# SaeedRahmani/MPC-RL_for_AVs

Hardware: AMD Instinct MI355X
Metric: MPC solves/sec (horizon=20, batch=4096) (higher is better)
Workload: dtype f64

## Files before the change

### mpc-rl_for_avs_amd/csrc/mpc_engine.hip

```cpp
#include <hip/hip_runtime.h>

#include <atomic>
#include <chrono>
#include <cmath>
#include <cstdio>
#include <cstring>
#include <new>
#include <string>
#include <vector>

#include "../../include/mpc_mi355x.h"
#include "mpc_core.hpp"
#include "mpc_ltv.hpp"
#include "mpc_wave.hpp"
#include "mpc_wave_dev.hpp"
#include "mpc_preamble.hpp"
#include "mpc_preamble_wave.hpp"
#include "mpc_synth_env.hpp"
#include "mpc_rollout_glue.hpp"

namespace {

thread_local std::string g_last_error;

int fail(int code, const std::string &msg) {
    g_last_error = msg;
    return code;
}

#define HIP_TRY(expr)                                                                              \
    do {                                                                                           \
        hipError_t e_ = (expr);                                                                    \
        if (e_ != hipSuccess)                                                                      \
            return fail(MPC_ERR_HIP, std::string(#expr) + ": " + hipGetErrorString(e_));          \
    } while (0)

constexpr int kBlock = 64;
constexpr int kMaxDevices = 64;
constexpr int kWaveOcc = 3, kWaveOccGeneric = 3;
constexpr int kWaveOccGenericCC = 2;
constexpr int kWaveOccLat = 2, kLatDepth = 4;
constexpr int kRelaxLat = 7;

template <int NC, int RELAX = 0>
struct WaveCtx : mpc::wave::WaveOpsT<RELAX> {
    static constexpr int kN = NC;
    const double *table;
    int e0, M;
    __device__ __forceinline__ WaveCtx(mpc::wave::lds_double_t *l, const double *t, int e, int m)
        : mpc::wave::WaveOpsT<RELAX>{l}, table(t), e0(e), M(m) {}
    __device__ __forceinline__ void tick(int) const {}
    __device__ __forceinline__ double ref(int k, int c) const {
        int idx = e0 + k;
        idx = idx > M - 1 ? M - 1 : idx;
        idx = idx < 0 ? 0 : idx;
        return table[idx * mpc::REF_COLS + c];
    }
    __device__ __forceinline__ double refv(int k) const {
        int idx = e0 + k;
        idx = idx > M - 1 ? M - 1 : idx;
        idx = idx < 0 ? 0 : idx;
        return table[M * mpc::REF_COLS + idx];
    }
};

template <bool CC, class CTX>
__device__ __forceinline__ void stage_problem(CTX &ctx, const mpc::SolveParams &P, int b, int lane, int N, int SL,
                                              const double *__restrict__ ref5, int M, const double *__restrict__ vref,
                                              const double *__restrict__ others, int Vin) {
    const int OTH = SL * (N + 1) + mpc::wave::SC_SIZE;
    for (int node = lane; node <= N; node += kBlock) {
        double rv;
        if (vref) {
            rv = vref[(size_t)b * (N + 1) + node];
        } else {
            int idx = ctx.e0 + node;
            idx = idx > M - 1 ? M - 1 : idx;
            idx = idx < 0 ? 0 : idx;
            rv = ref5[M * mpc::REF_COLS + idx];
        }
        ctx.st(node * SL + mpc::wave::W_RV, rv);
    }
    if (CC && lane < P.V) {
        const double *ov = others + ((size_t)b * Vin + lane) * 4;
        const double sp = ov[2] * P.dt, hh = ov[3];
        ctx.st(OTH + lane * 4 + 0, ov[0]);
        ctx.st(OTH + lane * 4 + 1, ov[1]);
        ctx.st(OTH + lane * 4 + 2, sp * cos(hh));
        ctx.st(OTH + lane * 4 + 3, sp * sin(hh));
    }
}

template <bool CC, int NC, int OCC, int RELAX>
__global__ __launch_bounds__(kBlock, OCC) void mpc_solve_wave_kernel(
    mpc::SolveParams P, int B, const double *__restrict__ ref5, int M, const double *__restrict__ state,
    const int32_t *__restrict__ ego_index, const double *__restrict__ vref, const double *__restrict__ weights,
    const uint8_t *__restrict__ is_collide, const double *__restrict__ others, int Vin,
    const int32_t *__restrict__ nveh, double w_collision, const double *u_init, int u_shift, uint8_t *u_valid,
    double *__restrict__ u0_out, double *U_out, double *__restrict__ X_out, int32_t *__restrict__ status_out,
// ... 1486 lines not shown
```

### mpc-rl_for_avs_amd/csrc/mpc_wave.hpp

```cpp
#pragma once

#include "mpc_core.hpp"

namespace mpc {
namespace wave {

constexpr int kLanes = 64;
constexpr int kTrials = 4;
constexpr double kProjKeep = 0.1;
constexpr double kProjKeepEnd = 1e-3, kProjEndMu = 1e-6;
constexpr int kGnWatch = 4, kGnSkip = 4;
constexpr double kGnEndMu = 1e-2;
constexpr int kDwProbe = 4;
constexpr int kBoostIter = 28;
constexpr double kOpenLoopStep = 1e-9;
constexpr double kAcceptableTol = 1e-6;
constexpr int kAcceptableIter = 15;
constexpr double kRegMax = 1.0;
constexpr double kKappaEps = 30.0;
constexpr double kMinSlack = 1e-14;
constexpr double kInitPush = 1e-2;

enum : int {
    W_X = 0,
// ... 7 lines not shown
    W_KX = 36,
    W_KP = 44,
    W_KF = 48,
    W_RV = 50,
    W_ONE = 51,
    W_DTC = 52,
    W_SLOTS = 53,
    W_LX = 53,
    W_Q = 55,
    W_QG = 58,
    W_ZW = 61,
    W_WJ = 62,
    W_CROSS = 63,
    W_SLOTS_CC = 65
};
constexpr int kZeroWord = W_LIN + 2;
enum : int { LIN_A02 = 0, LIN_A12 = 1, LIN_A03 = 4, LIN_A13 = 5, LIN_A23 = 6, LIN_B01 = 8, LIN_B11 = 9, LIN_B21 = 10 };
enum : int { W_DXY = W_LX, W_GW = W_Q, W_DZW = W_Q + 1 };
static_assert(kTrials == 4, "the trial areas below are laid out for four trials");
MPC_HD constexpr int trial_x(bool, int t, int TB) { return t == 0 ? TB : (t == 1 ? W_LIN : (t == 2 ? W_LIN + 6 : W_KX)); }
MPC_HD constexpr int trial_u(bool cc, int t, int TB) { return trial_x(cc, t, TB); }
enum : int {
    SC_SPARE = 0,
    SC_TRIG = 4,
    SC_LOG = SC_TRIG + kTrigWords,
    SC_BND = SC_LOG + kLogWords,
    SC_K = SC_BND + 8,
    SC_NB = SC_K + 6,
    SC_SIZE = SC_NB + 3
};
enum : int { K_SF = 0, K_RD, K_RC, K_QTT, K_Q33, K_MUMIN };
constexpr int kMaxHorizon = kLanes;
enum : int {
    A_L00 = W_KX + 0, A_L01 = W_KX + 1, A_L11 = W_KX + 2, A_H22 = W_KX + 3, A_H23 = W_KX + 4, A_H33 = W_KX + 5,
    A_WTD = W_KX + 6, A_WVD = W_KX + 7, A_H66 = W_KP + 0, A_H77 = W_KP + 1, A_HV6 = W_KP + 2, A_HV7 = W_KF + 0,
    A_HV4 = W_KF + 1,
    A_HV0 = W_X,
    A_HV5 = W_U
};

constexpr int kPreSlots = 12;
enum : int { PQ = 0, PB = 8 };
constexpr double kNoBound = 1e300;

MPC_HD constexpr int stage_slots(bool cc) { return (cc ? W_SLOTS_CC : W_SLOTS) + kPreSlots; }
MPC_HD constexpr int lds_doubles(bool cc, int N, int V) { return stage_slots(cc) * (N + 1) + SC_SIZE + (cc ? 4 * V : 0); }

enum : int {
    T_PREP = 0, T_ADJOINT, T_DUALRES, T_RIC_INIT, T_RIC_SCALARS, T_RIC_L1, T_RIC_L2, T_RIC_2X2, T_RIC_L4, T_LINEAR,
    T_RATIOS, T_ROLL_DYN, T_ROLL_COST, T_DUALUPD,
    T_R_FEEDBACK, T_R_CLAMP, T_R_DYN, T_R_STORE, T_R_CHECK, T_R_PROJ, T_R_LDSW, T_COUNT
};
template <class CTX, class = void>
struct fine_ticks { static constexpr bool value = false; };
template <class CTX>
struct fine_ticks<CTX, decltype((void)CTX::kFine)> { static constexpr bool value = CTX::kFine; };

template <class T>
struct PerLane {
#if defined(__HIPCC__)
    T v;
    MPC_HD T &at(int) { return v; }
#else
    T v[kLanes];
    MPC_HD T &at(int lane) { return v[lane]; }
#endif
};

MPC_HD bool ratio_greater(double n2, double d2, double n1, double d1) {
    const double a = n2 * d1, b = n1 * d2;
    return a > b || (a == b && d2 > d1);
}

#if !defined(__HIPCC__)
inline int row_partner(int l, int step) {
    return step == 0 ? (l ^ 1) : (step == 1 ? (l ^ 2) : (step == 2 ? ((l & ~7) | (7 - (l & 7))) : ((l & ~15) | (15 - (l & 15)))));
}
template <class T, class OP>
inline void host_row_reduce(PerLane<T> &p, OP op) {
    for (int step = 0; step < 4; ++step) {
        T nv[kLanes];
        for (int l = 0; l < kLanes; ++l) nv[l] = op(p.v[l], p.v[row_partner(l, step)]);
        for (int l = 0; l < kLanes; ++l) p.v[l] = nv[l];
    }
}
template <class T, class OP>
inline T host_reduce(PerLane<T> &p, OP op) {
    host_row_reduce(p, op);
    return op(op(p.v[0], p.v[16]), op(p.v[32], p.v[48]));
}
#endif

MPC_HD constexpr int stage_transition_word(int r, int c, int lin, int zero, int one, int dtw) {
    const int key = 8 * r + c;
    int w = zero;
    w = (r < 4 && r == c) ? one : w;
    w = key == 8 * 4 + 6 ? one : w;
    w = key == 8 * 5 + 7 ? one : w;
    w = key == 8 * 0 + 2 ? lin + 0 : w;
    w = key == 8 * 0 + 3 ? lin + 1 : w;
    w = key == 8 * 1 + 2 ? lin + 2 : w;
    w = key == 8 * 1 + 3 ? lin + 3 : w;
    w = key == 8 * 2 + 3 ? lin + 4 : w;
    w = key == 8 * 3 + 6 ? dtw : w;
    w = key == 8 * 0 + 7 ? lin + 5 : w;
    w = key == 8 * 1 + 7 ? lin + 6 : w;
// ... 15 lines not shown
    MPC_HD double RC() const { return sc(SC_K + K_RC); }
    MPC_HD double WS() const { return c.fresh(ws_); }
    MPC_HD double WC() const { return c.fresh(wc_); }
    MPC_HD double WD() const { return c.fresh(wd_); }
    MPC_HD double WCOLL() const { return c.fresh(wcoll); }

    MPC_HD Solver(const SolveParams &P_, CTX &c_, const double *x0_, double ws, double wc, double wd, double wcl)
        : P(P_), c(c_), N(CTX::kN > 0 ? CTX::kN : P_.N), SL(stage_slots(CC)), SCR(SL * (N + 1)), OTH(SCR + SC_SIZE),
          dt(P_.dt), ws_(c_.uni(ws)), wc_(c_.uni(wc)), wd_(c_.uni(wd)), wcoll(c_.uni(wcl)) {
        x0[0] = x0_[0]; x0[1] = x0_[1]; x0[2] = x0_[2]; x0[3] = x0_[3];
    }
    MPC_HD double S(int k, int slot) const { return c.ld(k * SL + slot); }
    MPC_HD void S(int k, int slot, double v) { c.st(k * SL + slot, v); }
    MPC_HD double sc(int i) const { return c.ld(SCR + i); }
    MPC_HD void sc(int i, double v) { c.st(SCR + i, v); }
    MPC_HD double oth(int j, int q) const { return c.ld(OTH + j * 4 + q); }
    MPC_HD double xlo(int i) const { return sc(SC_BND + 0 + 2 * i); }
    MPC_HD double xhi(int i) const { return sc(SC_BND + 1 + 2 * i); }
    MPC_HD double ulo(int i) const { return sc(SC_BND + 4 + 2 * i); }
    MPC_HD double uhi(int i) const { return sc(SC_BND + 5 + 2 * i); }
    MPC_HD double flog(double x) const {
        double K[kLogWords];
        for (int i = 0; i < kLogWords; ++i) K[i] = sc(SC_LOG + i);
        return log_pos(K, x);
    }
    MPC_HD TrigCoef trig() const {
        TrigCoef K;
        for (int i = 0; i < 6; ++i) {
            K.s[i] = sc(SC_TRIG + i);
            K.c[i] = sc(SC_TRIG + 6 + i);
        }
        return K;
    }

    PerLane<double> red_a, red_b, red_c, red_w;
    PerLane<int> ls_feas;
    int any_wall = 0;
    MPC_HD int f_word(int r, int c) const {
        const int w = stage_transition_word(r, c, 0, 1000, 1001, 1002);
        int t = w;
        t = w == 1000 ? kZeroWord : t;
        t = w == 1001 ? W_ONE : t;
        t = w == 1002 ? W_DTC : t;
        t = w == 0 ? W_LIN + LIN_A02 : t;
        t = w == 1 ? W_LIN + LIN_A03 : t;
        t = w == 2 ? W_LIN + LIN_A12 : t;
        t = w == 3 ? W_LIN + LIN_A13 : t;
        t = w == 4 ? W_LIN + LIN_A23 : t;
        t = w == 5 ? W_LIN + LIN_B01 : t;
        t = w == 6 ? W_LIN + LIN_B11 : t;
        t = w == 7 ? W_LIN + LIN_B21 : t;
        return t;
    }
    PerLane<int> r_a, r_b, r_lxx, r_lux, r_m, r_lx, r_lu, r_kx;
    MPC_HD void set_roles4(int AB) {
        c.lanes([&](int lane_) {
            const int lane = c.opaque(lane_);
            const int hi = lane >> 4, blk = (lane >> 2) & 3, lo = lane & 3;
            const int zero = kZeroWord;
            r_a.at(lane_) = f_word(hi, lo);
            r_b.at(lane_) = f_word(hi, lo < 2 ? 6 + lo : 4);
            const int a = hi < lo ? hi : lo, b = hi < lo ? lo : hi;
            const int key = a * 4 + b;
            int slot = zero;
            slot = key == 0 * 4 + 0 ? A_L00 : slot;
            slot = key == 0 * 4 + 1 ? A_L01 : slot;
            slot = key == 1 * 4 + 1 ? A_L11 : slot;
            slot = key == 2 * 4 + 2 ? A_H22 : slot;
            slot = key == 2 * 4 + 3 ? A_H23 : slot;
            slot = key == 3 * 4 + 3 ? A_H33 : slot;
            r_lxx.at(lane_) = slot;
            r_lux.at(lane_) = hi == 1 ? (lo == 2 ? A_WTD : (lo == 3 ? A_WVD : zero)) : zero;
            r_m.at(lane_) = (hi == 0 && lo == 0) ? A_H66 : ((hi == 1 && lo == 1) ? A_H77 : zero);
            r_lx.at(lane_) = lo == 0 ? AB + A_HV0 + hi : zero;
            r_lu.at(lane_) = lo == 0 ? (hi == 0 ? A_HV6 : (hi == 1 ? A_HV7 : zero)) : zero;
            int out = -1;
            out = (blk == 0 && hi < 2) ? W_KX + 2 * lo + hi : out;
            out = (blk == 1 && hi < 2 && lo < 2) ? W_KP + 2 * lo + hi : out;
            out = (blk == 2 && hi < 2 && lo == 0) ? W_KF + hi : out;
            r_kx.at(lane_) = out;
        });
    }

    MPC_HD void load_stage4(int k, int AB, PerLane<double> &RA, PerLane<double> &RB, PerLane<double> &QXX, PerLane<double> &QUX,
                            PerLane<double> &M, PerLane<double> &QX, PerLane<double> &QU, double &lp0, double &lp1) {
        c.lanes([&](int lane) {
            const int base = k * SL;
            auto word = [&](int w) { return c.ld(base + w); };
            RA.at(lane) = word(r_a.at(lane));
            RB.at(lane) = word(r_b.at(lane));
            QXX.at(lane) = word(r_lxx.at(lane));
            QUX.at(lane) = word(r_lux.at(lane));
            M.at(lane) = word(r_m.at(lane));
            QX.at(lane) = word(r_lx.at(lane));
            QU.at(lane) = word(r_lu.at(lane));
        });
        lp0 = S(k, A_HV4);
        lp1 = S(k, AB + A_HV5);
    }
    MPC_HD bool sweep4(int CB, int AB, double mu, double delta_w, bool gn, double &dV1) {
        double tsig[2], tgr[2];
        for (int i = 0; i < 2; ++i) {
            const double xi = S(N, CB + W_X + 2 + i);
            const double rl = frcp(xi - xlo(i)), ru = frcp(xhi(i) - xi);
            tsig[i] = S(N, W_ZXL + i) * rl + S(N, W_ZXU + i) * ru + delta_w;
            tgr[i] = mu * (ru - rl);
        }
        PerLane<double> PXX, PXP, PX;
        c.lanes([&](int lane_) {
            const int lane = c.opaque_shared(lane_);
            const int hi = lane >> 4, lo = lane & 3;
            PXX.at(lane_) = hi == lo ? (hi == 2 ? tsig[0] : (hi == 3 ? tsig[1] : delta_w)) : 0.0;
            PXP.at(lane_) = 0.0;
            PX.at(lane_) = lo == 0 ? (hi == 2 ? tgr[0] : (hi == 3 ? tgr[1] : 0.0)) : 0.0;
        });
        double pp00 = 0.0, pp01 = 0.0, pp11 = 0.0, ppv0 = 0.0, ppv1 = 0.0;
        c.tick(T_RIC_INIT);
        const double rd_full = RD();
#pragma unroll 1
        for (int k = N - 1; k >= 0; --k) {
            const double rdk = (k >= 1) ? rd_full : 0.0;
            PerLane<double> RA, RB, QXX, QUX, M, QX, QU, T0, T1;
            double lp0, lp1;
            load_stage4(k, AB, RA, RB, QXX, QUX, M, QX, QU, lp0, lp1);
            c.lanes([&](int lane) {
                T0.at(lane) = 0.0;
// ... 67 lines not shown
                            q11 = S(k, W_QG + 2) - S(k, W_Q + 2);
                            if (any_wall && S(k, W_WJ) >= 0.0) {
                                q00 += 2.0 * S(k, W_ZW);
                                q11 += 2.0 * S(k, W_ZW);
                            }
                        }
                    }
                }
                c.lanes([&](int lane_) {
                    const int lane = c.opaque_shared(lane_);
                    const int hi = lane >> 4, lo = lane & 3;
                    const int a = hi < lo ? hi : lo, b = hi < lo ? lo : hi;
                    double cx = 0.0;
                    switch (a * 4 + b) {
                        case 0 * 4 + 0: cx = q00; break;
                        case 0 * 4 + 1: cx = q01; break;
                        case 1 * 4 + 1: cx = q11; break;
                        case 2 * 4 + 2: cx = -wtt; break;
                        case 2 * 4 + 3: cx = -wtv; break;
                        default: break;
                    }
                    QXX.at(lane_) += cx;
                    QUX.at(lane_) += hi == 1 ? (lo == 2 ? -wtd : (lo == 3 ? -wvd : 0.0)) : 0.0;
                });
                hc -= wdd;
                det = ha * hc - hb * hb;
                pd = (ha > 0.0) & (hc > 0.0) & (det > c.fresh(1e-12) * ha * hc);
                if (pd) stage_tail();
            }
            if (!pd) return false;
            c.tick(T_RIC_2X2);
            dV1 += 0.5 * (kf0 * hu0 + kf1 * hu1);
            const double kp00 = rdk * i00, kp01 = rdk * i01, kp11 = rdk * i11;
            c.lanes([&](int lane) {
                PXX.at(lane) = PXXn.at(lane);
                PXP.at(lane) = PXPn.at(lane);
                PX.at(lane) = PXn.at(lane);
                const int ks = r_kx.at(lane);
                const bool is_kp = (ks >= W_KP) & (ks < W_KF), is_kf = ks >= W_KF;
                const double t = is_kf ? KFB.at(lane) : (is_kp ? -NWA.at(lane) : Ya.at(lane));
                const double v = (idet * t) * (is_kp ? rd_full : 1.0);
                if (ks >= 0) S(k, ks, v);
            });
            pp00 = rdk - rdk * kp00;
            pp01 = -rdk * kp01;
            pp11 = rdk - rdk * kp11;
            ppv0 = lp0 - rdk * kf0;
            ppv1 = lp1 - rdk * kf1;
            c.tick(T_RIC_L4);
        }
        return true;
    }

    MPC_HD double track(int k, double x_0, double x_1, double x_2, double x_3, double *g) const {
        const double s = c.ref(k, R_SIN), cc = c.ref(k, R_COS);
        const double dx = x_0 - c.ref(k, R_X), dy = x_1 - c.ref(k, R_Y);
        const double perp = dx * s - dy * cc, para = dx * cc + dy * s;
        const double dv = x_3 - S(k, W_RV), dth = x_2 - c.ref(k, R_H);
        if (g) {
            g[0] = 10.0 * (8.0 * perp * s + 4.0 * para * cc);
            g[1] = 10.0 * (-8.0 * perp * cc + 4.0 * para * s);
            g[2] = 10.0 * dth;
            g[3] = 20.0 * WS() * dv;
        }
        return 10.0 * (4.0 * perp * perp + 2.0 * para * para + WS() * dv * dv + 0.5 * dth * dth);
    }
    MPC_HD double dist(int k, double x_0, double x_1, double *d8, int j0 = 0, int dj = 1) const {
        double J = 0.0, g0 = 0, g1 = 0, h00 = 0, h01 = 0, h11 = 0, c00 = 0, c01 = 0, c11 = 0;
        for (int j = j0; j < P.V; j += dj) {
            const double px = x_0 - (oth(j, 0) + k * oth(j, 2));
            const double py = x_1 - (oth(j, 1) + k * oth(j, 3));
            const double d2 = fma(px, px, py * py);
            const double rd = frsqrt(d2), d = d2 * rd;
            const double cst = (d2 < 1.0 ? c.fresh(1000.0) : c.fresh(100.0)) * P.w_distance;
            const double rde = frcp(d + c.fresh(1e-6));
            const double inv2 = rde * rde;
            J += cst * inv2;
            if (d8) {
                const double dpsi = -2.0 * cst * inv2 * rde;
                const double nx = px * rd, ny = py * rd;
                const double d2psi = 6.0 * cst * inv2 * inv2;
                const double tt = dpsi * rd;
                g0 += dpsi * nx;
                g1 += dpsi * ny;
                h00 += d2psi * nx * nx + tt * (1.0 - nx * nx);
                h01 += (d2psi - tt) * nx * ny;
                h11 += d2psi * ny * ny + tt * (1.0 - ny * ny);
                c00 += d2psi * nx * nx;
                c01 += d2psi * nx * ny;
                c11 += d2psi * ny * ny;
            }
        }
        if (d8) {
            d8[0] = g0; d8[1] = g1; d8[2] = h00; d8[3] = h01; d8[4] = h11; d8[5] = c00; d8[6] = c01; d8[7] = c11;
        }
        return J;
    }
    MPC_HD double wall_slack(int k, double x_0, double x_1, int j, double &nx, double &ny) const {
        const double px = x_0 - (oth(j, 0) + k * oth(j, 2));
        const double py = x_1 - (oth(j, 1) + k * oth(j, 3));
        nx = 2.0 * px;
        ny = 2.0 * py;
        return fma(px, px, py * py) - 1.0;
    }
    MPC_HD void cost_grad(int cb, int k, double *lx) const {
        const int B = cb * 6;
// ... 755 lines not shown
                    r1 -= rd_full * (S(k + 1, CB + W_U + 1) - u1);
                }
                const double b01 = S(k, W_LIN + LIN_B01), b11 = S(k, W_LIN + LIN_B11), b21 = S(k, W_LIN + LIN_B21);
                r0 += dt * S(k + 1, W_Y + 3);
                r1 += b01 * S(k + 1, W_Y + 0) + b11 * S(k + 1, W_Y + 1) + b21 * S(k + 1, W_Y + 2);
                red_a.at(lane) = fmax2(fabs(r0), fabs(r1));
            });
            const double err_d = c.wave_max(red_a);
            const double s_d = fmax2(100.0, (sum_lam + sum_z) / (10.0 * N)) / 100.0;
            const double s_c = fmax2(100.0, sum_z / (6.0 * N)) / 100.0;
            for (;;) {
                const double ec = fmax2(cmax - mu, mu - cmin);
                const double E_mu = fmax2(err_d / s_d, ec / s_c);
                if (E_mu <= c.fresh(kKappaEps) * mu && mu > sc(SC_K + K_MUMIN)) {
                    mu = c.uni(fmax2(sc(SC_K + K_MUMIN), fmin2(c.fresh(0.2) * mu, mu * sqrt(mu))));
                    continue;
                }
                break;
            }
            const double E0 = fmax2(err_d / s_d, cmax / s_c);
            kkt_out = E0;
            if (E0 <= P.tol) {
                status_out = (CC && zw_max > c.fresh(1e-6) * SF()) ? 5 : 0;
                break;
            }
            if (P.tol < kAcceptableTol) {
                n_acceptable = (E0 <= c.fresh(kAcceptableTol)) ? n_acceptable + 1 : 0;
                if (n_acceptable >= kAcceptableIter) {
                    status_out = (CC && zw_max > c.fresh(1e-6) * SF()) ? 7 : 6;
                    break;
                }
            }
            if (iter == P.max_iter) break;
            if (P.stall_window > 0) {
                if (E0 < 0.5 * e_mark) {
                    e_mark = c.uni(E0);
                    i_mark = iter;
                } else if (iter - i_mark >= P.stall_window) {
                    status_out = 4;
                    break;
                }
            }

            c.tick(T_DUALRES);
            const int AB = (cur ^ 1) * 6;
            double dV1 = 0.0, delta_w = reg;
            bool ok = false, gn = false;
            int nmod = 0;
            if (nonconvex_cost && prev_needed && iter % kDwProbe != 0) {
                delta_w = fmax2(reg, c.fresh(1.0 / 3.0) * c.uni(sc(SC_SPARE + 3)));
                gn = prev_gn && !(mu <= c.fresh(kGnEndMu));
            }
            bool skipped_gn = false;
            set_roles4(AB);
            for (int attempt = 0; attempt < 16 && !ok; ++attempt) {
                ok = true;
                dV1 = 0.0;
                c.phase([&](int lane) {
                    if (lane >= N) return;
                    const int k = lane;
                    const double rc = RC(), qtt = sc(SC_K + K_QTT), q33 = sc(SC_K + K_Q33);
                    const double rdk = (k >= 1) ? RD() : 0.0;
                    const double v = S(k, CB + W_X + 3);
                    const double u0 = S(k, CB + W_U + 0), u1 = S(k, CB + W_U + 1);
                    double sig[4], sgr[4];
                    for (int q = 0; q < 4; ++q) {
                        const bool isx = q < 2;
                        const int b = isx ? q : q - 2;
                        const double val = isx ? S(k, CB + W_X + 2 + b) : (b == 0 ? u0 : u1);
                        const double lo = isx ? xlo(b) : ulo(b), hi = isx ? xhi(b) : uhi(b);
                        const double zl = isx ? S(k, W_ZXL + b) : S(k, W_ZUL + b);
                        const double zu = isx ? S(k, W_ZXU + b) : S(k, W_ZUU + b);
                        const double rl = frcp(val - lo), ru = frcp(hi - val);
                        sig[q] = zl * rl + zu * ru;
                        sgr[q] = mu * (ru - rl);
                    }
                    double wdd = 0.0, wtt = 0.0, wtv = 0.0, wtd = 0.0, wvd = 0.0;
                    if (!gn) {
                        double Sn, Cn, sb, cb_, bp, bpp;
                        dyn_eval(trig(), S(k, CB + W_X + 2), u1, Sn, Cn, sb, cb_);
                        beta_derivs(sb, cb_, bp, bpp);
                        const double yy0 = S(k + 1, W_Y + 0), yy1 = S(k + 1, W_Y + 1), yy2 = S(k + 1, W_Y + 2);
                        const double g = -(yy0 * Cn + yy1 * Sn), h = -(yy0 * Sn - yy1 * Cn);
                        wdd = dt * v * (g * bp * bp + h * bpp) + dt * yy2 * v * kInvWheelbase * (-sb * bp * bp + cb_ * bpp);
                        wtt = dt * v * g;
                        wtv = dt * h;
                        wtd = dt * v * g * bp;
                        wvd = dt * h * bp + dt * yy2 * cb_ * bp * kInvWheelbase;
                    }
                    double l00 = 0.0, l01 = 0.0, l11 = 0.0, h22 = 0.0, h23 = 0.0, h33 = 0.0, hv0 = 0.0, hv1 = 0.0, hv2 = 0.0,
                           hv3 = 0.0;
                    if (k >= 1) {
                        double lx[4];
                        cost_grad(cur, k, lx);
                        const double s = c.ref(k, R_SIN), cc = c.ref(k, R_COS);
                        l00 = SF() * 10.0 * (8.0 * s * s + 4.0 * cc * cc) + delta_w;
                        l01 = SF() * 10.0 * (-8.0 * s * cc + 4.0 * cc * s);
                        l11 = SF() * 10.0 * (8.0 * cc * cc + 4.0 * s * s) + delta_w;
                        if (CC) {
                            const int QS = gn ? W_QG : W_Q;
                            l00 += S(k, QS + 0);
                            l01 += S(k, QS + 1);
                            l11 += S(k, QS + 2);
                        }
                        h22 = wtt + qtt + sig[0] + delta_w;
                        h23 = wtv;
                        h33 = q33 + sig[1] + delta_w;
                        hv0 = lx[0];
                        hv1 = lx[1];
                        if (CC && any_wall) {
                            const double wjv = S(k, W_WJ);
                            if (wjv >= 0.0) {
                                double nx, ny;
                                const double rg = frcp(wall_slack(k, S(k, CB + W_X + 0), S(k, CB + W_X + 1), (int)wjv, nx, ny));
                                const double zw = S(k, W_ZW), sg = zw * rg, cv = gn ? 0.0 : 2.0 * zw;
                                l00 += sg * nx * nx - cv;
                                l01 += sg * nx * ny;
                                l11 += sg * ny * ny - cv;
                                hv0 -= mu * rg * nx;
                                hv1 -= mu * rg * ny;
                            }
                        }
                        hv2 = lx[2] + sgr[0];
                        hv3 = lx[3] + sgr[1];
                    } else {
                        wtd = 0.0;
                        wvd = 0.0;
                    }
                    double um0 = 0.0, um1 = 0.0;
                    if (k >= 1) {
                        um0 = S(k - 1, CB + W_U + 0);
                        um1 = S(k - 1, CB + W_U + 1);
                    }
                    S(k, A_L00, l00);
                    S(k, A_L01, l01);
                    S(k, A_L11, l11);
                    S(k, A_H22, h22);
                    S(k, A_H23, h23);
                    S(k, A_H33, h33);
                    S(k, A_WTD, wtd);
                    S(k, A_WVD, wvd);
                    S(k, A_H66, rc + rdk + sig[2] + delta_w);
                    S(k, A_H77, rc + rdk + sig[3] + delta_w + wdd);
                    S(k, AB + A_HV0, hv0);
                    S(k, AB + A_HV0 + 1, hv1);
                    S(k, AB + A_HV0 + 2, hv2);
                    S(k, AB + A_HV0 + 3, hv3);
                    S(k, A_HV4, -rdk * (u0 - um0));
                    S(k, AB + A_HV5, -rdk * (u1 - um1));
                    S(k, A_HV6, rc * u0 + rdk * (u0 - um0) + sgr[2]);
                    S(k, A_HV7, rc * u1 + rdk * (u1 - um1) + sgr[3]);
                });
                ok = sweep4(CB, AB, mu, delta_w, gn, dV1);
                if (!ok) {
                    ++nmod;
                    if (gn_skip > 0) skipped_gn = true;
                    if (!gn && gn_skip == 0 && !(nonconvex_cost && mu <= c.fresh(kGnEndMu))) {
                        gn = true;
                    } else {
                        const double dw_last = c.uni(sc(SC_SPARE + 3));
                        if (dw_last == 0.0) {
                            delta_w = (delta_w < 1e-4) ? c.fresh(1e-4) : c.fresh(100.0) * delta_w;
                        } else {
                            const double third = c.fresh(1.0 / 3.0) * dw_last;
                            delta_w = (delta_w < third) ? third : c.fresh(8.0) * delta_w;
                        }
                    }
                    if (delta_w > 1e40) break;
                }
            }
            if (!ok) {
                status_out = 2;
                break;
            }
            if (delta_w > reg) sc(SC_SPARE + 3, delta_w);
            prev_needed = delta_w > reg;
            prev_gn = gn;
            if (nmod > 0) {
                if (gn_streak == 0) e_streak = c.uni(E0);
                ++gn_streak;
                if (gn_skip > 0) {
                    --gn_skip;
                } else if (gn_streak % kGnWatch == 0) {
                    if (E0 > 0.5 * e_streak) gn_skip = kGnSkip;
                    e_streak = c.uni(E0);
                }
            } else {
                gn_streak = 0;
                gn_skip = 0;
            }

            c.tick(T_RIC_INIT);
            const double tau = c.uni(fmax2(0.99, 1.0 - mu));
            c.tick(T_LINEAR);
            if (CC && any_wall) {
                c.phase([&](int lane) {
                    const int kn = lane + 1;
                    if (kn >= N) return;
                    const double wjv = S(kn, W_WJ);
                    if (wjv >= 0.0) {
                        double nx, ny;
                        S(kn, W_GW, wall_slack(kn, S(kn, CB + W_X + 0), S(kn, CB + W_X + 1), (int)wjv, nx, ny));
                    }
                });
            }
            const double phi0 = c.uni(Jcur + mu * barcur);
            const int tb = cur ^ 1;
            double Jn = 0.0, barn = 0.0;
            int acc_trial = -1;
            const double keep = c.uni(mu <= c.fresh(kProjEndMu) ? c.fresh(kProjKeepEnd) : c.fresh(kProjKeep));
            const bool accepted = line_search(cur, 0.5 * (1.0 - tau), keep, phi0, dV1, mu, Jn, barn, acc_trial);
            const bool have_cross = CC && P.V > 0 && acc_trial != 0;
            c.phase([&](int lane) {
                if (lane >= N) {
                    red_b.at(lane) = 0.0;
                    red_c.at(lane) = 1.0;
                    return;
                }
                const int k = lane;
                double rdn = 0.0, rdd = 1.0;
// ... 123 lines not shown
```

Measured before the change: 1.058 million.

## Add dual-candidate Riccati sweep to factor two regularization trials per wave

```diff
diff --git a/mpc-rl_for_avs_amd/csrc/mpc_engine.hip b/mpc-rl_for_avs_amd/csrc/mpc_engine.hip
--- a/mpc-rl_for_avs_amd/csrc/mpc_engine.hip
+++ b/mpc-rl_for_avs_amd/csrc/mpc_engine.hip
@@ -45,6 +45,7 @@
 template <int NC, int RELAX = 0>
 struct WaveCtx : mpc::wave::WaveOpsT<RELAX> {
     static constexpr int kN = NC;
+    static constexpr int kDualMode = (RELAX & 4) ? 1 : 0;
     const double *table;
     int e0, M;
     __device__ __forceinline__ WaveCtx(mpc::wave::lds_double_t *l, const double *t, int e, int m)
diff --git a/mpc-rl_for_avs_amd/csrc/mpc_wave.hpp b/mpc-rl_for_avs_amd/csrc/mpc_wave.hpp
--- a/mpc-rl_for_avs_amd/csrc/mpc_wave.hpp
+++ b/mpc-rl_for_avs_amd/csrc/mpc_wave.hpp
@@ -83,6 +83,14 @@
     T_R_FEEDBACK, T_R_CLAMP, T_R_DYN, T_R_STORE, T_R_CHECK, T_R_PROJ, T_R_LDSW, T_COUNT
 };
 template <class CTX, class = void>
+struct dual_mode { static constexpr int value = 0; };
+template <class CTX>
+struct dual_mode<CTX, decltype((void)CTX::kDualMode)> { static constexpr int value = CTX::kDualMode; };
+template <class CTX>
+MPC_HD auto note_sweep(CTX &c, int which, int) -> decltype((void)c.sweeps[0]) { ++c.sweeps[which]; }
+template <class CTX>
+MPC_HD void note_sweep(CTX &, int, long) {}
+template <class CTX, class = void>
 struct fine_ticks { static constexpr bool value = false; };
 template <class CTX>
 struct fine_ticks<CTX, decltype((void)CTX::kFine)> { static constexpr bool value = CTX::kFine; };
@@ -204,12 +212,14 @@
         t = w == 7 ? W_LIN + LIN_B21 : t;
         return t;
     }
+    static constexpr int kDualOff = (CC ? W_SLOTS_CC : W_SLOTS) - W_KX;
     PerLane<int> r_a, r_b, r_lxx, r_lux, r_m, r_lx, r_lu, r_kx;
+    template <bool DUAL = false>
     MPC_HD void set_roles4(int AB) {
         c.lanes([&](int lane_) {
             const int lane = c.opaque(lane_);
             const int hi = lane >> 4, blk = (lane >> 2) & 3, lo = lane & 3;
-            const int zero = kZeroWord;
+            const int zero = kZeroWord, hoff = (DUAL && blk >= 2) ? kDualOff : 0;
             r_a.at(lane_) = f_word(hi, lo);
             r_b.at(lane_) = f_word(hi, lo < 2 ? 6 + lo : 4);
             const int a = hi < lo ? hi : lo, b = hi < lo ? lo : hi;
@@ -221,9 +231,9 @@
             slot = key == 2 * 4 + 2 ? A_H22 : slot;
             slot = key == 2 * 4 + 3 ? A_H23 : slot;
             slot = key == 3 * 4 + 3 ? A_H33 : slot;
-            r_lxx.at(lane_) = slot;
-            r_lux.at(lane_) = hi == 1 ? (lo == 2 ? A_WTD : (lo == 3 ? A_WVD : zero)) : zero;
-            r_m.at(lane_) = (hi == 0 && lo == 0) ? A_H66 : ((hi == 1 && lo == 1) ? A_H77 : zero);
+            r_lxx.at(lane_) = slot == zero ? zero : slot + hoff;
+            r_lux.at(lane_) = hi == 1 ? (lo == 2 ? A_WTD + hoff : (lo == 3 ? A_WVD + hoff : zero)) : zero;
+            r_m.at(lane_) = (hi == 0 && lo == 0) ? A_H66 + hoff : ((hi == 1 && lo == 1) ? A_H77 + hoff : zero);
             r_lx.at(lane_) = lo == 0 ? AB + A_HV0 + hi : zero;
             r_lu.at(lane_) = lo == 0 ? (hi == 0 ? A_HV6 : (hi == 1 ? A_HV7 : zero)) : zero;
             int out = -1;
@@ -397,6 +407,309 @@
         return true;
     }
 
+    MPC_HD int sweep4_dual(int CB, int AB, double mu, double dwA, bool gnA, double dwB, bool gnB, double &dV1A, double &dV1B) {
+        double tsA[2], tsB[2], tgr[2];
+        for (int i = 0; i < 2; ++i) {
+            const double xi = S(N, CB + W_X + 2 + i);
+            const double rl = frcp(xi - xlo(i)), ru = frcp(xhi(i) - xi);
+            const double zs = S(N, W_ZXL + i) * rl + S(N, W_ZXU + i) * ru;
+            tsA[i] = zs + dwA;
+            tsB[i] = zs + dwB;
+            tgr[i] = mu * (ru - rl);
+        }
+        PerLane<double> PXX, PXP, PX, P00, P01, P11, PV0, PV1, DV;
+        c.lanes([&](int lane_) {
+            const int lane = c.opaque_shared(lane_);
+            const int hi = lane >> 4, lo = lane & 3;
+            const bool mb = ((lane >> 2) & 3) >= 2;
+            const double t0 = mb ? tsB[0] : tsA[0], t1 = mb ? tsB[1] : tsA[1], dw = mb ? dwB : dwA;
+            PXX.at(lane_) = hi == lo ? (hi == 2 ? t0 : (hi == 3 ? t1 : dw)) : 0.0;
+            PXP.at(lane_) = 0.0;
+            PX.at(lane_) = lo == 0 ? (hi == 2 ? tgr[0] : (hi == 3 ? tgr[1] : 0.0)) : 0.0;
+            P00.at(lane_) = 0.0;
+            P01.at(lane_) = 0.0;
+            P11.at(lane_) = 0.0;
+            PV0.at(lane_) = 0.0;
+            PV1.at(lane_) = 0.0;
+            DV.at(lane_) = 0.0;
+        });
+        bool aliveA = true, aliveB = true;
+        c.tick(T_RIC_INIT);
+        const double rd_full = RD();
+#pragma unroll 1
+        for (int k = N - 1; k >= 0; --k) {
+            const double rdk = (k >= 1) ? rd_full : 0.0;
+            PerLane<double> RA, RB, QXX, QUX, M, QX, QU, T0, T1;
+            double lp0, lp1;
+            load_stage4(k, AB, RA, RB, QXX, QUX, M, QX, QU, lp0, lp1);
+            c.lanes([&](int lane) {
+                T0.at(lane) = 0.0;
+                T1.at(lane) = PXP.at(lane);
+            });
+            c.tick(T_RIC_SCALARS);
+            c.mfma(PXX, RA, T0);
+            c.mfma(PXX, RB, T1);
+            c.mfma(PXP, RB, M);
+            c.mfma(RA, PX, QX);
+            c.mfma(RB, PX, QU);
+            c.tick(T_RIC_L1);
+            c.mfma(RB, T1, M);
+            c.mfma(T1, RA, QUX);
+            c.mfma(RA, T0, QXX);
+            c.tick(T_RIC_L2);
+            const double mA0 = c.lane_get(M, 0), mA1 = c.lane_get(M, 1), mA2 = c.lane_get(M, 17);
+            const double mB0 = c.lane_get(M, 8), mB1 = c.lane_get(M, 9), mB2 = c.lane_get(M, 25);
+            const double uA0 = c.lane_get(QU, 0), uA1 = c.lane_get(QU, 16), uB0 = c.lane_get(QU, 8), uB1 = c.lane_get(QU, 24);
+            PerLane<double> HA, HB, HC, HU0, HU1, DET;
+            PerLane<int> PD;
+            c.lanes([&](int lane_) {
+                const bool mb = ((c.opaque_shared(lane_) >> 2) & 3) >= 2;
+                const double ha = (mb ? mB0 : mA0) + P00.at(lane_), hb = (mb ? mB1 : mA1) + P01.at(lane_);
+                const double hc = (mb ? mB2 : mA2) + P11.at(lane_);
+                const double det = ha * hc - hb * hb;
+                HA.at(lane_) = ha;
+                HB.at(lane_) = hb;
+                HC.at(lane_) = hc;
+                HU0.at(lane_) = (mb ? uB0 : uA0) + PV0.at(lane_);
+                HU1.at(lane_) = (mb ? uB1 : uA1) + PV1.at(lane_);
+                DET.at(lane_) = det;
+                PD.at(lane_) = (ha > 0.0) & (hc > 0.0) & (det > c.fresh(1e-12) * ha * hc);
+            });
+            bool pdA = c.wave_bcast(PD, 0) != 0, pdB = c.wave_bcast(PD, 8) != 0;
+            PerLane<double> NWA, RWA, Ya, QS, KFB, IDET, PXXn, PXPn, PXn;
+            auto stage_tail = [&]() {
+                c.lanes([&](int lane_) {
+                    const int lane = c.opaque_shared(lane_);
+                    const int hi = lane >> 4, lo = lane & 3;
+                    const double ha = HA.at(lane_), hb = HB.at(lane_), hc = HC.at(lane_);
+                    const double hu0 = HU0.at(lane_), hu1 = HU1.at(lane_);
+                    const double kfa0 = hb * hu1 - hc * hu0, kfa1 = hb * hu0 - ha * hu1;
+                    const double w00 = (hi == 0 && lo == 0) ? 1.0 : 0.0, w11 = (hi == 1 && lo == 1) ? 1.0 : 0.0;
+                    const double wof = ((hi == 0 && lo == 1) || (hi == 1 && lo == 0)) ? 1.0 : 0.0;
+                    const double c1 = (hi == 1 && lo == 0) ? 1.0 : 0.0;
+                    const double nwa = wof * hb - w00 * hc - w11 * ha;
+                    NWA.at(lane_) = nwa;
+                    RWA.at(lane_) = -rdk * nwa;
+                    KFB.at(lane_) = w00 * kfa0 + c1 * kfa1;
+                    Ya.at(lane_) = 0.0;
+                    PXPn.at(lane_) = 0.0;
+                    PXXn.at(lane_) = QXX.at(lane_);
+                    PXn.at(lane_) = QX.at(lane_);
+                });
+                c.mfma(NWA, QUX, Ya);
+                c.lanes([&](int lane_) {
+                    const double idet = frcp(DET.at(lane_));
+                    IDET.at(lane_) = idet;
+                    QS.at(lane_) = idet * QUX.at(lane_);
+                });
+                c.mfma(QS, Ya, PXXn);
+                c.mfma(QS, RWA, PXPn);
+                c.mfma(QS, KFB, PXn);
+            };
+            stage_tail();
+            const bool fbA = aliveA && !pdA && !gnA, fbB = aliveB && !pdB && !gnB;
+            if (fbA || fbB) {
+                double wdd, wtt = 0.0, wtv = 0.0, wtd = 0.0, wvd = 0.0, q00 = 0.0, q01 = 0.0, q11 = 0.0;
+                {
+                    const double v = S(k, CB + W_X + 3);
+                    double Sn, Cn, sb, cb_, bp, bpp;
+                    dyn_eval(trig(), S(k, CB + W_X + 2), S(k, CB + W_U + 1), Sn, Cn, sb, cb_);
+                    beta_derivs(sb, cb_, bp, bpp);
+                    const double yy0 = S(k + 1, W_Y + 0), yy1 = S(k + 1, W_Y + 1), yy2 = S(k + 1, W_Y + 2);
+                    const double g = -(yy0 * Cn + yy1 * Sn), h = -(yy0 * Sn - yy1 * Cn);
+                    wdd = dt * v * (g * bp * bp + h * bpp) + dt * yy2 * v * kInvWheelbase * (-sb * bp * bp + cb_ * bpp);
+                    if (k >= 1) {
+                        wtt = dt * v * g;
+                        wtv = dt * h;
+                        wtd = dt * v * g * bp;
+                        wvd = dt * h * bp + dt * yy2 * cb_ * bp * kInvWheelbase;
+                        if (CC) {
+                            q00 = S(k, W_QG + 0) - S(k, W_Q + 0);
+                            q01 = S(k, W_QG + 1) - S(k, W_Q + 1);
+                            q11 = S(k, W_QG + 2) - S(k, W_Q + 2);
+                            if (any_wall && S(k, W_WJ) >= 0.0) {
+                                q00 += 2.0 * S(k, W_ZW);
+                                q11 += 2.0 * S(k, W_ZW);
+                            }
+                        }
+                    }
+                }
+                c.lanes([&](int lane_) {
+                    const int lane = c.opaque_shared(lane_);
+                    const int hi = lane >> 4, lo = lane & 3;
+                    if (!((((lane >> 2) & 3) >= 2) ? fbB : fbA)) return;
+                    const int a = hi < lo ? hi : lo, b = hi < lo ? lo : hi;
+                    double cx = 0.0;
+                    switch (a * 4 + b) {
+                        case 0 * 4 + 0: cx = q00; break;
+                        case 0 * 4 + 1: cx = q01; break;
+                        case 1 * 4 + 1: cx = q11; break;
+                        case 2 * 4 + 2: cx = -wtt; break;
+                        case 2 * 4 + 3: cx = -wtv; break;
+                        default: break;
+                    }
+                    QXX.at(lane_) += cx;
+                    QUX.at(lane_) += hi == 1 ? (lo == 2 ? -wtd : (lo == 3 ? -wvd : 0.0)) : 0.0;
+                    const double ha = HA.at(lane_), hb = HB.at(lane_), hc = HC.at(lane_) - wdd;
+                    const double det = ha * hc - hb * hb;
+                    HC.at(lane_) = hc;
+                    DET.at(lane_) = det;
+                    PD.at(lane_) = (ha > 0.0) & (hc > 0.0) & (det > c.fresh(1e-12) * ha * hc);
+                });
+                if (fbA) pdA = c.wave_bcast(PD, 0) != 0;
+                if (fbB) pdB = c.wave_bcast(PD, 8) != 0;
+                if ((fbA && pdA) || (fbB && pdB)) stage_tail();
+            }
+            aliveA = aliveA && pdA;
+            aliveB = aliveB && pdB;
+            if (!aliveA && !aliveB) return 0;
+            c.tick(T_RIC_2X2);
+            c.lanes([&](int lane_) {
+                PXX.at(lane_) = PXXn.at(lane_);
+                PXP.at(lane_) = PXPn.at(lane_);
+                PX.at(lane_) = PXn.at(lane_);
+                const int lane = c.opaque_shared(lane_);
+                const int hi = lane >> 4, blk = (lane >> 2) & 3, lo = lane & 3;
+                const bool mb = blk >= 2, is_kp = (blk & 1) != 0;
+                const double idet = IDET.at(lane_);
+                const int off = mb ? kDualOff : 0;
+                if (hi < 2 && (!is_kp || lo < 2)) {
+                    const double t = is_kp ? -NWA.at(lane_) : Ya.at(lane_);
+                    S(k, off + (is_kp ? W_KP : W_KX) + 2 * lo + hi, (idet * t) * (is_kp ? rd_full : 1.0));
+                }
+                if (is_kp && hi < 2 && lo == 0) S(k, (mb ? AB + W_X : W_KF) + hi, idet * KFB.at(lane_));
+                const double ha = HA.at(lane_), hb = HB.at(lane_), hc = HC.at(lane_);
+                const double hu0 = HU0.at(lane_), hu1 = HU1.at(lane_);
+                const double kf0 = (hb * hu1 - hc * hu0) * idet, kf1 = (hb * hu0 - ha * hu1) * idet;
+                DV.at(lane_) += 0.5 * (kf0 * hu0 + kf1 * hu1);
+                const double kp00 = rdk * (hc * idet), kp01 = rdk * (-hb * idet), kp11 = rdk * (ha * idet);
+                P00.at(lane_) = rdk - rdk * kp00;
+                P01.at(lane_) = -rdk * kp01;
+                P11.at(lane_) = rdk - rdk * kp11;
+                PV0.at(lane_) = lp0 - rdk * kf0;
+                PV1.at(lane_) = lp1 - rdk * kf1;
+            });
+            c.tick(T_RIC_L4);
+        }
+        dV1A = c.lane_get(DV, 0);
+        dV1B = c.lane_get(DV, 8);
+        return aliveA ? 1 : 2;
+    }
+    MPC_HD void dual_take_b(int AB) {
+        c.phase([&](int lane) {
+            if (lane >= N) return;
+            const int k = lane;
+            for (int i = 0; i < 12; ++i) S(k, W_KX + i, S(k, W_KX + kDualOff + i));
+            S(k, W_KF + 0, S(k, AB + W_X + 0));
+            S(k, W_KF + 1, S(k, AB + W_X + 1));
+        });
+    }
+
+    template <bool DUAL>
+    MPC_HD void assemble(int cur, int AB, double mu, bool gnA, double dwA, bool gnB = false, double dwB = 0.0) {
+        const int CB = cur * 6;
+        c.phase([&](int lane) {
+            const bool mb = DUAL && lane >= 32;
+            const int k = DUAL ? (lane & 31) : lane;
+            if (k >= N) return;
+            const bool gn = mb ? gnB : gnA;
+            const double delta_w = mb ? dwB : dwA;
+            auto SH = [&](int slot, double v) { S(k, mb ? slot + kDualOff : slot, v); };
+            const double rc = RC(), qtt = sc(SC_K + K_QTT), q33 = sc(SC_K + K_Q33);
+            const double rdk = (k >= 1) ? RD() : 0.0;
+            const double v = S(k, CB + W_X + 3);
+            const double u0 = S(k, CB + W_U + 0), u1 = S(k, CB + W_U + 1);
+            double sig[4], sgr[4];
+            for (int q = 0; q < 4; ++q) {
+                const bool isx = q < 2;
+                const int b = isx ? q : q - 2;
+                const double val = isx ? S(k, CB + W_X + 2 + b) : (b == 0 ? u0 : u1);
+                const double lo = isx ? xlo(b) : ulo(b), hi = isx ? xhi(b) : uhi(b);
+                const double zl = isx ? S(k, W_ZXL + b) : S(k, W_ZUL + b);
+                const double zu = isx ? S(k, W_ZXU + b) : S(k, W_ZUU + b);
+                const double rl = frcp(val - lo), ru = frcp(hi - val);
+                sig[q] = zl * rl + zu * ru;
+                sgr[q] = mu * (ru - rl);
+            }
+            double wdd = 0.0, wtt = 0.0, wtv = 0.0, wtd = 0.0, wvd = 0.0;
+            if (!gn) {
+                double Sn, Cn, sb, cb_, bp, bpp;
+                dyn_eval(trig(), S(k, CB + W_X + 2), u1, Sn, Cn, sb, cb_);
+                beta_derivs(sb, cb_, bp, bpp);
+                const double yy0 = S(k + 1, W_Y + 0), yy1 = S(k + 1, W_Y + 1), yy2 = S(k + 1, W_Y + 2);
+                const double g = -(yy0 * Cn + yy1 * Sn), h = -(yy0 * Sn - yy1 * Cn);
+                wdd = dt * v * (g * bp * bp + h * bpp) + dt * yy2 * v * kInvWheelbase * (-sb * bp * bp + cb_ * bpp);
+                wtt = dt * v * g;
+                wtv = dt * h;
+                wtd = dt * v * g * bp;
+                wvd = dt * h * bp + dt * yy2 * cb_ * bp * kInvWheelbase;
+            }
+            double l00 = 0.0, l01 = 0.0, l11 = 0.0, h22 = 0.0, h23 = 0.0, h33 = 0.0, hv0 = 0.0, hv1 = 0.0, hv2 = 0.0,
+                   hv3 = 0.0;
+            if (k >= 1) {
+                double lx[4];
+                cost_grad(cur, k, lx);
+                const double s = c.ref(k, R_SIN), cc = c.ref(k, R_COS);
+                l00 = SF() * 10.0 * (8.0 * s * s + 4.0 * cc * cc) + delta_w;
+                l01 = SF() * 10.0 * (-8.0 * s * cc + 4.0 * cc * s);
+                l11 = SF() * 10.0 * (8.0 * cc * cc + 4.0 * s * s) + delta_w;
+                if (CC) {
+                    const int QS = gn ? W_QG : W_Q;
+                    l00 += S(k, QS + 0);
+                    l01 += S(k, QS + 1);
+                    l11 += S(k, QS + 2);
+                }
+                h22 = wtt + qtt + sig[0] + delta_w;
+                h23 = wtv;
+                h33 = q33 + sig[1] + delta_w;
+                hv0 = lx[0];
+                hv1 = lx[1];
+                if (CC && any_wall) {
+                    const double wjv = S(k, W_WJ);
+                    if (wjv >= 0.0) {
+                        double nx, ny;
+                        const double rg = frcp(wall_slack(k, S(k, CB + W_X + 0), S(k, CB + W_X + 1), (int)wjv, nx, ny));
+                        const double zw = S(k, W_ZW), sg = zw * rg, cv = gn ? 0.0 : 2.0 * zw;
+                        l00 += sg * nx * nx - cv;
+                        l01 += sg * nx * ny;
+                        l11 += sg * ny * ny - cv;
+                        hv0 -= mu * rg * nx;
+                        hv1 -= mu * rg * ny;
+                    }
+                }
+                hv2 = lx[2] + sgr[0];
+                hv3 = lx[3] + sgr[1];
+            } else {
+                wtd = 0.0;
+                wvd = 0.0;
+            }
+            double um0 = 0.0, um1 = 0.0;
+            if (k >= 1) {
+                um0 = S(k - 1, CB + W_U + 0);
+                um1 = S(k - 1, CB + W_U + 1);
+            }
+            SH(A_L00, l00);
+            SH(A_L01, l01);
+            SH(A_L11, l11);
+            SH(A_H22, h22);
+            SH(A_H23, h23);
+            SH(A_H33, h33);
+            SH(A_WTD, wtd);
+            SH(A_WVD, wvd);
+            SH(A_H66, rc + rdk + sig[2] + delta_w);
+            SH(A_H77, rc + rdk + sig[3] + delta_w + wdd);
+            if (mb) return;
+            S(k, AB + A_HV0, hv0);
+            S(k, AB + A_HV0 + 1, hv1);
+            S(k, AB + A_HV0 + 2, hv2);
+            S(k, AB + A_HV0 + 3, hv3);
+            S(k, A_HV4, -rdk * (u0 - um0));
+            S(k, AB + A_HV5, -rdk * (u1 - um1));
+            S(k, A_HV6, rc * u0 + rdk * (u0 - um0) + sgr[2]);
+            S(k, A_HV7, rc * u1 + rdk * (u1 - um1) + sgr[3]);
+        });
+    }
+
     MPC_HD double track(int k, double x_0, double x_1, double x_2, double x_3, double *g) const {
         const double s = c.ref(k, R_SIN), cc = c.ref(k, R_COS);
         const double dx = x_0 - c.ref(k, R_X), dy = x_1 - c.ref(k, R_Y);
@@ -1258,120 +1571,62 @@
                 gn = prev_gn && !(mu <= c.fresh(kGnEndMu));
             }
             bool skipped_gn = false;
+            auto next_model = [&](bool &gn_, double &dw_) {
+                if (!gn_ && gn_skip == 0 && !(nonconvex_cost && mu <= c.fresh(kGnEndMu))) {
+                    gn_ = true;
+                } else {
+                    const double dw_last = c.uni(sc(SC_SPARE + 3));
+                    if (dw_last == 0.0) {
+                        dw_ = (dw_ < 1e-4) ? c.fresh(1e-4) : c.fresh(100.0) * dw_;
+                    } else {
+                        const double third = c.fresh(1.0 / 3.0) * dw_last;
+                        dw_ = (dw_ < third) ? third : c.fresh(8.0) * dw_;
+                    }
+                }
+            };
             set_roles4(AB);
-            for (int attempt = 0; attempt < 16 && !ok; ++attempt) {
+            int attempt = 0;
+            if constexpr (dual_mode<CTX>::value != 0) {
+                bool gnB = gn;
+                double dwB = delta_w;
+                next_model(gnB, dwB);
+                if ((dual_mode<CTX>::value == 2 || gn_streak > 0) && N <= 32 && !(dwB > 1e40)) {
+                    set_roles4<true>(AB);
+                    assemble<true>(cur, AB, mu, gn, delta_w, gnB, dwB);
+                    double dV1B = 0.0;
+                    const int r = sweep4_dual(CB, AB, mu, delta_w, gn, dwB, gnB, dV1, dV1B);
+                    note_sweep(c, 1, 0);
+                    attempt = r == 1 ? 1 : 2;
+                    if (r == 1) {
+                        ok = true;
+                    } else {
+                        ++nmod;
+                        if (gn_skip > 0) skipped_gn = true;
+                        gn = gnB;
+                        delta_w = dwB;
+                        if (r == 2) {
+                            ok = true;
+                            dV1 = dV1B;
+                            dual_take_b(AB);
+                        } else {
+                            ++nmod;
+                            next_model(gn, delta_w);
+                            if (delta_w > 1e40) attempt = 16;
+                            set_roles4(AB);
+                        }
+                    }
+                }
+            }
+            for (; attempt < 16 && !ok; ++attempt) {
                 ok = true;
                 dV1 = 0.0;
-                c.phase([&](int lane) {
-                    if (lane >= N) return;
-                    const int k = lane;
-                    const double rc = RC(), qtt = sc(SC_K + K_QTT), q33 = sc(SC_K + K_Q33);
-                    const double rdk = (k >= 1) ? RD() : 0.0;
-                    const double v = S(k, CB + W_X + 3);
-                    const double u0 = S(k, CB + W_U + 0), u1 = S(k, CB + W_U + 1);
-                    double sig[4], sgr[4];
-                    for (int q = 0; q < 4; ++q) {
-                        const bool isx = q < 2;
-                        const int b = isx ? q : q - 2;
-                        const double val = isx ? S(k, CB + W_X + 2 + b) : (b == 0 ? u0 : u1);
-                        const double lo = isx ? xlo(b) : ulo(b), hi = isx ? xhi(b) : uhi(b);
-                        const double zl = isx ? S(k, W_ZXL + b) : S(k, W_ZUL + b);
-                        const double zu = isx ? S(k, W_ZXU + b) : S(k, W_ZUU + b);
-                        const double rl = frcp(val - lo), ru = frcp(hi - val);
-                        sig[q] = zl * rl + zu * ru;
-                        sgr[q] = mu * (ru - rl);
-                    }
-                    double wdd = 0.0, wtt = 0.0, wtv = 0.0, wtd = 0.0, wvd = 0.0;
-                    if (!gn) {
-                        double Sn, Cn, sb, cb_, bp, bpp;
-                        dyn_eval(trig(), S(k, CB + W_X + 2), u1, Sn, Cn, sb, cb_);
-                        beta_derivs(sb, cb_, bp, bpp);
-                        const double yy0 = S(k + 1, W_Y + 0), yy1 = S(k + 1, W_Y + 1), yy2 = S(k + 1, W_Y + 2);
-                        const double g = -(yy0 * Cn + yy1 * Sn), h = -(yy0 * Sn - yy1 * Cn);
-                        wdd = dt * v * (g * bp * bp + h * bpp) + dt * yy2 * v * kInvWheelbase * (-sb * bp * bp + cb_ * bpp);
-                        wtt = dt * v * g;
-                        wtv = dt * h;
-                        wtd = dt * v * g * bp;
-                        wvd = dt * h * bp + dt * yy2 * cb_ * bp * kInvWheelbase;
-                    }
-                    double l00 = 0.0, l01 = 0.0, l11 = 0.0, h22 = 0.0, h23 = 0.0, h33 = 0.0, hv0 = 0.0, hv1 = 0.0, hv2 = 0.0,
-                           hv3 = 0.0;
-                    if (k >= 1) {
-                        double lx[4];
-                        cost_grad(cur, k, lx);
-                        const double s = c.ref(k, R_SIN), cc = c.ref(k, R_COS);
-                        l00 = SF() * 10.0 * (8.0 * s * s + 4.0 * cc * cc) + delta_w;
-                        l01 = SF() * 10.0 * (-8.0 * s * cc + 4.0 * cc * s);
-                        l11 = SF() * 10.0 * (8.0 * cc * cc + 4.0 * s * s) + delta_w;
-                        if (CC) {
-                            const int QS = gn ? W_QG : W_Q;
-                            l00 += S(k, QS + 0);
-                            l01 += S(k, QS + 1);
-                            l11 += S(k, QS + 2);
-                        }
-                        h22 = wtt + qtt + sig[0] + delta_w;
-                        h23 = wtv;
-                        h33 = q33 + sig[1] + delta_w;
-                        hv0 = lx[0];
-                        hv1 = lx[1];
-                        if (CC && any_wall) {
-                            const double wjv = S(k, W_WJ);
-                            if (wjv >= 0.0) {
-                                double nx, ny;
-                                const double rg = frcp(wall_slack(k, S(k, CB + W_X + 0), S(k, CB + W_X + 1), (int)wjv, nx, ny));
-                                const double zw = S(k, W_ZW), sg = zw * rg, cv = gn ? 0.0 : 2.0 * zw;
-                                l00 += sg * nx * nx - cv;
-                                l01 += sg * nx * ny;
-                                l11 += sg * ny * ny - cv;
-                                hv0 -= mu * rg * nx;
-                                hv1 -= mu * rg * ny;
-                            }
-                        }
-                        hv2 = lx[2] + sgr[0];
-                        hv3 = lx[3] + sgr[1];
-                    } else {
-                        wtd = 0.0;
-                        wvd = 0.0;
-                    }
-                    double um0 = 0.0, um1 = 0.0;
-                    if (k >= 1) {
-                        um0 = S(k - 1, CB + W_U + 0);
-                        um1 = S(k - 1, CB + W_U + 1);
-                    }
-                    S(k, A_L00, l00);
-                    S(k, A_L01, l01);
-                    S(k, A_L11, l11);
-                    S(k, A_H22, h22);
-                    S(k, A_H23, h23);
-                    S(k, A_H33, h33);
-                    S(k, A_WTD, wtd);
-                    S(k, A_WVD, wvd);
-                    S(k, A_H66, rc + rdk + sig[2] + delta_w);
-                    S(k, A_H77, rc + rdk + sig[3] + delta_w + wdd);
-                    S(k, AB + A_HV0, hv0);
-                    S(k, AB + A_HV0 + 1, hv1);
-                    S(k, AB + A_HV0 + 2, hv2);
-                    S(k, AB + A_HV0 + 3, hv3);
-                    S(k, A_HV4, -rdk * (u0 - um0));
-                    S(k, AB + A_HV5, -rdk * (u1 - um1));
-                    S(k, A_HV6, rc * u0 + rdk * (u0 - um0) + sgr[2]);
-                    S(k, A_HV7, rc * u1 + rdk * (u1 - um1) + sgr[3]);
-                });
+                assemble<false>(cur, AB, mu, gn, delta_w);
                 ok = sweep4(CB, AB, mu, delta_w, gn, dV1);
+                note_sweep(c, 0, 0);
                 if (!ok) {
                     ++nmod;
                     if (gn_skip > 0) skipped_gn = true;
-                    if (!gn && gn_skip == 0 && !(nonconvex_cost && mu <= c.fresh(kGnEndMu))) {
-                        gn = true;
-                    } else {
-                        const double dw_last = c.uni(sc(SC_SPARE + 3));
-                        if (dw_last == 0.0) {
-                            delta_w = (delta_w < 1e-4) ? c.fresh(1e-4) : c.fresh(100.0) * delta_w;
-                        } else {
-                            const double third = c.fresh(1.0 / 3.0) * dw_last;
-                            delta_w = (delta_w < third) ? third : c.fresh(8.0) * delta_w;
-                        }
-                    }
+                    next_model(gn, delta_w);
                     if (delta_w > 1e40) break;
                 }
             }
```

New measurement: 1.084 million, median of 6. 1.02x the previous value.
